# imironhead/ml_super_resolution

Measured on AMD Instinct MI355X. Metric: VDSR-20 training patches/sec (41x41, batch 256 per GPU); fwd HR megapixels/sec alongside, higher is better.
Workload: dtype f32; 1 GPU; BASELINE configs[2]: VDSR 20-layer 3x3x64 residual, RGB, batch 256x41x41 per GPU, fwd+bwd+TF-Adam, random-init weights; global_batch=256, patch=41, parallelism=dp1

## Files before the change

### include/srx.h

```cpp
#ifndef SRX_H_
#define SRX_H_

#include <stddef.h>
#include <stdint.h>

#ifdef __cplusplus
extern "C" {
#endif

typedef void* srx_stream_t;

typedef enum {
    SRX_OK = 0,
    SRX_ERR_BAD_ARG = -1,
    SRX_ERR_UNSUPPORTED = -2,
    SRX_ERR_WORKSPACE = -3,
    SRX_ERR_LAUNCH = -4,
    SRX_ERR_ALIGN = -5
} srx_status;

typedef enum { SRX_PAD_SAME = 0, SRX_PAD_VALID = 1 } srx_pad_mode;

typedef enum {
    SRX_ACT_NONE = 0,
// ... 42 lines not shown
                        const float* x_in, int in_act, float* dx_out, void* ws, size_t ws_bytes,
                        srx_stream_t stream);

int srx_conv2d_bwd_data_acc(const srx_conv_desc* d, const float* dpre, const float* w, const float* dx_acc,
                            float* dx_out, void* ws, size_t ws_bytes, srx_stream_t stream);

int srx_conv2d_bwd_filter(const srx_conv_desc* d, const float* x, const float* dpre, float* dw,
                          float* dbias, const float* w_for_decay, float wd_scale, void* ws,
                          size_t ws_bytes, srx_stream_t stream);

int srx_conv2d_bwd_filter_partials(const srx_conv_desc* d, const float* x, const float* dpre, void* ws,
                                   size_t ws_bytes, int* n_partials, srx_stream_t stream);
int srx_conv2d_bwd_filter_reduce(const srx_conv_desc* d, const void* ws, int n_partials, float* dw,
                                 float* dbias, const float* w_for_decay, float wd_scale,
                                 srx_stream_t stream);

int srx_act_bwd(const float* dy, const float* y, float* dpre, size_t numel, int act,
                srx_stream_t stream);

int srx_depth_to_space(const float* in, float* out, int N, int H, int W, int C, int r,
                       srx_stream_t stream);

int srx_stream_copy(const void* in, void* out, size_t bytes, srx_stream_t stream);

int srx_espcn_forward(const float* x, const float* w1, const float* b1, const float* w2, const float* b2,
                      const float* w3, const float* b3, float* hr, int N, int H, int W, int r,
                      srx_stream_t stream);
int srx_espcn_forward_keep(const float* x, const float* w1, const float* b1, const float* w2, const float* b2,
                           const float* w3, const float* b3, float* t1, float* t2, float* y, int N, int H, int W, int r,
                           srx_stream_t stream);
// ... 139 lines not shown
```

### ml_super_resolution_amd/_lib.py

```python
import ctypes
import os

_HERE = os.path.dirname(os.path.abspath(__file__))
LIB_PATH = os.path.join(_HERE, 'libsrx.so')

SRX_OK = 0
PAD_SAME, PAD_VALID = 0, 1
ACT_NONE, ACT_RELU, ACT_TANH, ACT_LRELU, ACT_SIGMOID = 0, 1, 2, 3, 4
OP_FWD, OP_BWD_DATA, OP_BWD_FILTER = 0, 1, 2
PRECISION_FP32, PRECISION_BF16X3 = 0, 1
PRECISION_BY_NAME = {'highest': PRECISION_FP32, 'high': PRECISION_BF16X3}

ACT_BY_NAME = {None: ACT_NONE, 'none': ACT_NONE, 'relu': ACT_RELU, 'tanh': ACT_TANH,
               'lrelu': ACT_LRELU, 'leaky_relu': ACT_LRELU, 'sigmoid': ACT_SIGMOID}
PAD_BY_NAME = {'same': PAD_SAME, 'valid': PAD_VALID}

EXPORTS = [
    'srx_version', 'srx_last_error', 'srx_set_conv_path', 'srx_set_wgrad_path', 'srx_set_chain', 'srx_conv_chain', 'srx_conv_chain_supported', 'srx_conv2d_precision_supported', 'srx_conv2d_workspace_bytes', 'srx_conv2d_fwd',
    'srx_conv2d_bwd_data', 'srx_conv2d_bwd_filter', 'srx_conv2d_bwd_filter_partials', 'srx_conv2d_bwd_filter_reduce', 'srx_act_bwd', 'srx_depth_to_space',
    'srx_space_to_depth', 'srx_stream_copy', 'srx_mse_fwd_bwd', 'srx_l2_loss', 'srx_reduce_scratch_bytes',
    'srx_adam_tf_step', 'srx_adam_tf_step_dev', 'srx_momentum_clip_step', 'srx_rownorm_loss_fwd_bwd', 'srx_psnr', 'srx_ssim', 'srx_ssim_scratch_bytes', 'srx_saturate_u8', 'srx_affine', 'srx_u8_to_unit_float', 'srx_gaussian_blur', 'srx_resize_bilinear',
    'srx_upsample_nearest', 'srx_upsample_nearest_bwd', 'srx_add_relu_grad',
    'srx_conv2d_bwd_data_acc', 'srx_conv3x3_blocked', 'srx_conv3x3_blocked_bwd_filter_workspace_bytes', 'srx_conv3x3_blocked_bwd_filter',
    'srx_conv3x3_blocked_ex', 'srx_conv3x3_blocked_bwd_filter_ex_workspace_bytes', 'srx_conv3x3_blocked_bwd_filter_ex',
    'srx_espcn_forward', 'srx_espcn_forward_keep', 'srx_debug_poison_lds', 'srx_srcnn_forward', 'srx_maxpool2x2', 'srx_maxpool2x2_bwd', 'srx_maxpool2x2_bwd_masked', 'srx_subsample2', 'srx_subsample2_bwd',
    'srx_channel_blocks_to_nhwc', 'srx_nhwc_to_channel_blocks', 'srx_channel_normalize', 'srx_channel_normalize_bwd',
    'srx_extract_patches16', 'srx_texture_gram', 'srx_texture_gram_bwd', 'srx_pil_resample_ksize', 'srx_pil_resample_coeffs', 'srx_resample_u8', 'srx_u8_to_pm1', 'srx_log_loss', 'srx_vgg_preprocess', 'srx_add_scaled', 'srx_resize_bicubic_tf', 'srx_column_sums', 'srx_gemm_workspace_bytes', 'srx_gemm',
]


class SrxError(RuntimeError):
    pass


# ... 30 lines not shown
    L.srx_last_error.restype = ctypes.c_char_p
    L.srx_set_conv_path.argtypes = [i]
    L.srx_set_wgrad_path.argtypes = [i]
    L.srx_set_chain.argtypes = [i]
    L.srx_conv_chain_supported.argtypes = [dp, i, i]
    L.srx_conv_chain.argtypes = [dp, i, i, i, vp, vp, vp, vp, vp, vp]
    L.srx_conv2d_precision_supported.argtypes = [dp, i]
    L.srx_conv2d_workspace_bytes.argtypes = [dp, i]
    L.srx_conv2d_workspace_bytes.restype = sz
    L.srx_reduce_scratch_bytes.restype = sz
    L.srx_conv2d_fwd.argtypes = [dp, vp, vp, vp, vp, vp, vp, sz, vp]
    L.srx_conv2d_bwd_data.argtypes = [dp, vp, vp, vp, i, vp, vp, sz, vp]
    L.srx_conv2d_bwd_filter.argtypes = [dp, vp, vp, vp, vp, vp, f, vp, sz, vp]
    L.srx_conv2d_bwd_filter_partials.argtypes = [dp, vp, vp, vp, sz, ctypes.POINTER(ctypes.c_int), vp]
    L.srx_conv2d_bwd_filter_reduce.argtypes = [dp, vp, i, vp, vp, vp, f, vp]
    L.srx_act_bwd.argtypes = [vp, vp, vp, sz, i, vp]
    L.srx_depth_to_space.argtypes = [vp, vp, i, i, i, i, i, vp]
    L.srx_space_to_depth.argtypes = [vp, vp, i, i, i, i, i, vp]
    L.srx_stream_copy.argtypes = [vp, vp, sz, vp]
    L.srx_mse_fwd_bwd.argtypes = [vp, vp, sz, f, vp, i, vp, vp, vp]
    L.srx_l2_loss.argtypes = [vp, vp, sz, f, vp, i, vp, vp]
    L.srx_adam_tf_step.argtypes = [vp, vp, vp, vp, sz, f, f, f, f, ctypes.c_int64, f, vp]
    L.srx_adam_tf_step_dev.argtypes = [vp, vp, vp, vp, sz, vp, f, f, f, f, vp]
    L.srx_momentum_clip_step.argtypes = [vp, vp, vp, sz, f, f, f, f, vp]
    L.srx_rownorm_loss_fwd_bwd.argtypes = [vp, vp, sz, sz, vp, vp, vp, vp]
    L.srx_psnr.argtypes = [vp, vp, vp, i, sz, f, vp]
    L.srx_ssim.argtypes = [vp, vp, vp, i, i, i, i, f, vp, vp]
    L.srx_ssim_scratch_bytes.argtypes = [i]
    L.srx_ssim_scratch_bytes.restype = sz
    L.srx_saturate_u8.argtypes = [vp, vp, sz, vp]
# ... 54 lines not shown
```

### ml_super_resolution_amd/csrc/conv_kernels.hip.h

```cpp
#pragma once
#include <hip/hip_runtime.h>
#include <stdint.h>
#include <type_traits>

namespace srx {

typedef float f32x4 __attribute__((ext_vector_type(4)));

enum { ACT_NONE = 0, ACT_RELU = 1, ACT_TANH = 2, ACT_LRELU = 3, ACT_SIGMOID = 4 };

struct ConvArgs {
    const float* x;
    const float* w;
    const float* bias;
    const float* skip;
    const float* mask;
    float* y;
    int N, H, W, OH, OW, Cin, Cout;
    int pad_t, pad_l;
    int TH, TW, NTX, RS;
    int units_total;
    int act, post_relu, mask_act;
    float inv_rs;
    int stagger;
// ... 2441 lines not shown
        }
    }
    bsum += __shfl_xor(bsum, 16);
    bsum += __shfl_xor(bsum, 32);
    if (qpart == 0 && kq == 0 && co_ok) pw[(size_t)TAPS * a.Cin * a.Cout + co] = bsum;
}

template <int IMM>
__device__ __forceinline__ float dpre_fire_imm(__amdgpu_buffer_rsrc_t rsrc, int voff, int soff) {
    float b;
    asm volatile("buffer_load_dword %0, %1, %2, %3 offen offset:%4" : "=&a"(b) : "v"(voff), "s"(rsrc), "s"(soff), "n"(IMM) : "memory");
    return b;
}

template <int KH, int KW, int CINP, int NCH, int OWC>
__global__ __launch_bounds__(256, 1) void wgrad_rows_full_kernel(const WgradArgs a) {
    extern __shared__ __attribute__((aligned(16))) float lds[];
    constexpr int PS = Lds<CINP>::PS;
    constexpr int TAPS = KH * KW;
    constexpr int ROWS = TAPS * CINP;
    constexpr int Q = (ROWS + 63) / 64;
    constexpr int NQP = 4 / NCH;
    constexpr int QW = (Q + NQP - 1) / NQP;
    constexpr int TPP = CINP / 4, PPP = 256 / TPP;
    constexpr int SPR = OWC / 4;
    constexpr int THC = 3;
    constexpr int RSZ = OWC + 1;
    constexpr int COUTC = 64;
    constexpr int U = THC * SPR + 1;
    constexpr int JP = (RSZ + PPP - 1) / PPP;
    constexpr int NPASSES = (THC + KH - 1) * JP;
// ... 44 lines not shown
    SG.m_row = SG.m_last; SG.m_mid = ~0ull;
    const int colb = 16 * COUTC;
    const int lane_b = (kq * COUTC + co_c) * 4;
    const int vb0 = lane_b, vb1 = lane_b + 4 * colb, vb2 = lane_b + 8 * colb;
    const int vX = ((kq * OWC + OWC - 1) * COUTC + co_c) * 4;
    const int rowb = __builtin_amdgcn_readfirstlane(OWC * COUTC * 4);
    const int srow1 = rowb, srow2 = __builtin_amdgcn_readfirstlane(2 * rowb);

    f32x4 acc[QW][4];
#pragma unroll
    for (int k = 0; k < QW; ++k)
#pragma unroll
        for (int g = 0; g < 4; ++g) acc[k][g] = f32x4{0.f, 0.f, 0.f, 0.f};
    float bsum = 0.f;

    const long G_ = gridDim.x;
    const int u0 = (int)(((long)blockIdx.x * a.units_total) / G_);
    const int u1 = (int)(((long)(blockIdx.x + 1) * a.units_total) / G_);

    auto tile_of = [&](int uu_, int& n, int& h, int& th) {
        h = uu_ % a.OH;
        n = uu_ / a.OH;
        th = THC;
        if (a.OH - h < th) th = a.OH - h;
        if (u1 - uu_ < th) th = u1 - uu_;
    };
    auto stage_setup = [&](StageSeq& qi, StageSeq& qc, int h, int th, int buf, bool active) {
        const int left = __builtin_amdgcn_readfirstlane(active ? (th + KH - 1) * JP : 0);
        const int above = (a.pad_t > h) ? (a.pad_t - h) * JP : 0;
        qi.j = 0; qc.j = 0;
        qi.off = __builtin_amdgcn_readfirstlane((h - a.pad_t) * a.W * CINP * 4);
        qc.off = __builtin_amdgcn_readfirstlane(buf * buf_bytes);
        qi.left = left; qc.left = left;
        qi.thr = __builtin_amdgcn_readfirstlane(left - above);
        qc.thr = 0;
    };
    auto x_rsrc = [&](int n) {
        return uniform_rsrc(a.x + ((size_t)n * a.H * a.W - a.pad_l) * CINP, (a.H * a.W + a.pad_l) * CINP * 4);
    };
    auto b_rsrc = [&](int n, int h, int th) {
        return uniform_rsrc(a.dpre + ((size_t)n * a.OH + h) * a.OW * COUTC, th * a.OW * COUTC * 4);
    };

    float bcur[U], bnext[U];
    auto dpre_window_now = [&](__amdgpu_buffer_rsrc_t brs) {
#pragma unroll
        for (int i = 0; i < U; ++i) {
            if (i == U - 1) {
                bnext[i] = __builtin_bit_cast(float, __builtin_amdgcn_raw_buffer_load_b32(brs, vX, 0, 0));
            } else {
                const int r = i / SPR, j = i % SPR;
                const int vb = j < 4 ? vb0 : (j < 8 ? vb1 : vb2);
                bnext[i] = __builtin_bit_cast(float, __builtin_amdgcn_raw_buffer_load_b32(brs, vb + (j % 4) * colb, r * rowb, 0));
            }
        }
    };
// ... 109 lines not shown
        stage_tile_scalar<CINP, 6>(qi, qc, SG, xrs, voff_lane, wl_lane);
        lds_barrier();
        cur_buf ^= 1;
        u = un_;
        t_end += SRX_STAMP() - ts_e;
    }
#undef SRX_TAKE_OVER_B
#ifdef SRX_TRACE
    if (a.trace && lane == 0) {
        unsigned long long* tr = a.trace + ((size_t)blockIdx.x * 4 + wave) * 12;
        tr[0] = t_begin; tr[1] = SRX_STAMP(); tr[2] = t_loop; tr[3] = t_end; tr[4] = 0;
    }
#endif

    asm volatile("s_nop 15\n\ts_nop 7" ::: "memory");
    float* pw = a.part + (size_t)blockIdx.x * a.part_stride;
#pragma unroll
    for (int k = 0; k < QW; ++k) {
        const int q = qpart + k * NQP;
        if (q >= Q) continue;
#pragma unroll
        for (int g = 0; g < 4; ++g) {
#pragma unroll
            for (int r = 0; r < 4; ++r) {
                const int R = 64 * q + 4 * (4 * kq + r) + g;
                const int tap = R / CINP, ci = R % CINP;
                if (R < ROWS && ci < a.Cin && co_ok) pw[((size_t)tap * a.Cin + ci) * a.Cout + co] = acc[k][g][r];
            }
        }
    }
    bsum += __shfl_xor(bsum, 16);
    bsum += __shfl_xor(bsum, 32);
    if (qpart == 0 && kq == 0 && co_ok) pw[(size_t)TAPS * a.Cin * a.Cout + co] = bsum;
}

}
```

### ml_super_resolution_amd/csrc/launchers.h

```cpp
#pragma once
#include "conv_kernels.hip.h"

namespace srx {

struct ConvKey {
    int kh, kw, cinp, nch;
    bool wt;
};

bool launch_conv_k3c64(const ConvKey& k, const ConvArgs& a, int grid, size_t lds, hipStream_t s, hipError_t* err);
bool launch_conv_k3c32(const ConvKey& k, const ConvArgs& a, int grid, size_t lds, hipStream_t s, hipError_t* err);
bool launch_conv_c4(const ConvKey& k, const ConvArgs& a, int grid, size_t lds, hipStream_t s, hipError_t* err);
bool launch_conv_misc(const ConvKey& k, const ConvArgs& a, int grid, size_t lds, hipStream_t s, hipError_t* err);
bool launch_pipe_k3c64(const ConvKey& k, const ConvArgs& a, int grid, size_t lds, hipStream_t s, hipError_t* err);
bool launch_pipe_other(const ConvKey& k, const ConvArgs& a, int grid, size_t lds, hipStream_t s, hipError_t* err);
bool launch_wgrad_narrow(const ConvKey& k, const WgradArgs& a, int grid, hipStream_t s, hipError_t* err);
bool launch_conv_narrow(const ConvKey& k, const ConvArgs& a, hipStream_t s, hipError_t* err);
bool launch_conv_1x1(const ConvKey& k, const ConvArgs& a, long min_pixels, hipStream_t s, hipError_t* err);
bool launch_conv_rows3x3(const ConvKey& k, const ConvArgs& a, long min_pixels, hipStream_t s, hipError_t* err);
bool launch_conv_pack3(const ConvKey& k, const ConvArgs& a, long min_pixels, hipStream_t s, hipError_t* err);
bool launch_conv_kwrows(const ConvKey& k, const ConvArgs& a, long min_pixels, hipStream_t s, hipError_t* err);
bool launch_pipe_strip(const ConvKey& k, const ConvArgs& a, int grid, size_t lds, hipStream_t s, hipError_t* err);
bool launch_conv_generic(const ConvKey& k, const ConvArgs& a, int grid, size_t lds, hipStream_t s, hipError_t* err);
bool launch_wgrad(const ConvKey& k, const WgradArgs& a, int grid, size_t lds, hipStream_t s, hipError_t* err);
bool launch_wgrad_generic(const ConvKey& k, const WgradArgs& a, int grid, size_t lds, hipStream_t s, hipError_t* err);
bool launch_wgrad_lin(const ConvKey& k, const WgradArgs& a, int grid, size_t lds, hipStream_t s, hipError_t* err);
bool launch_wgrad_lin_pack3(const ConvKey& k, const WgradArgs& a, int grid, size_t lds, hipStream_t s, hipError_t* err);
bool launch_wgrad_lin_strip(const ConvKey& k, const WgradArgs& a, int grid, size_t lds, hipStream_t s, hipError_t* err);
bool launch_wgrad_pipe(const ConvKey& k, const WgradArgs& a, int grid, size_t lds, hipStream_t s, hipError_t* err);
bool launch_wgrad_kwcols(const ConvKey& k, const WgradArgs& a, int max_partials, long min_pixels, int* n_partials, hipStream_t s, hipError_t* err);
bool launch_wgrad_1x1(const ConvKey& k, const WgradArgs& a, int max_partials, int* n_partials, hipStream_t s, hipError_t* err);
bool launch_wgrad_rows_full(const ConvKey& k, const WgradArgs& a, int grid, size_t lds, hipStream_t s, hipError_t* err);
bool launch_wgrad_rows_strip(const ConvKey& k, const WgradArgs& a, int grid, size_t lds, hipStream_t s, hipError_t* err);
bool launch_wgrad_lin_pairs(const ConvKey& k, const WgradPairs& q, int grid, int pairs, bool strips, size_t lds, hipStream_t s, hipError_t* err);

__attribute__((weak)) hipError_t launch_conv_chain(bool wt, bool aux, const ConvArgs& a, const ChainPtrs& c, int grid, size_t lds, hipStream_t s);

hipError_t launch_reduce_partials(const float* part, int G, int stride, int wn, int cout, float* dw, float* dbias,
                                  const float* w, float wd, hipStream_t s);
hipError_t launch_reduce_partials_pairs(const float* part, int G, int stride, int wn, int cout, float* dw, float* dbias,
                                        int pairs, int cob, hipStream_t s);

template <typename K, typename A>
inline hipError_t launch_with_lds(K kernel, const A& a, int grid, size_t lds, hipStream_t s, int grid_y = 1) {
    static thread_local const void* configured[64];
    static thread_local int n_configured = 0;
    const void* fn = reinterpret_cast<const void*>(kernel);
    bool known = false;
    for (int i = 0; i < n_configured; ++i) known |= (configured[i] == fn);
    if (!known) {
        hipError_t e = hipFuncSetAttribute(fn, hipFuncAttributeMaxDynamicSharedMemorySize, 160 * 1024);
// ... 98 lines not shown
```

### ml_super_resolution_amd/csrc/srx_api.hip

```cpp
#include <math.h>
#include <stdarg.h>
#include <atomic>
#include <stdio.h>
#include <stdlib.h>
#include <string.h>

#include "../../include/srx.h"
#include "elementwise.h"
#include "launchers.h"
#include "bf16x3.h"

using namespace srx;

namespace {

thread_local char g_err[512] = "";

struct Knobs {
    int pipe_default, narrow, wgrad_lin, wgrad_pipe, wgrad_pipe_strip, wgrad_rows_full, wgrad_1x1, wgrad_pack3, kwrows_min_pixels, big_route_min_pixels, strip_d2s, conv_1x1_min_pixels, pack3_dgrad;
    int chain;
    unsigned long long* trace;
    int dbg;
};
int env_int(const char* name, int dflt) { const char* e = getenv(name); return e ? atoi(e) : dflt; }
Knobs read_knobs() {
    Knobs k;
    k.pipe_default = env_int("SRX_PIPE", 1);
    k.narrow = env_int("SRX_NARROW", 1);
    k.wgrad_lin = env_int("SRX_WGRAD_LIN", 1);
    k.wgrad_pipe = env_int("SRX_WGRAD_PIPE", 1);
    k.wgrad_pipe_strip = env_int("SRX_WGRAD_PIPE_STRIP", 1);
    k.kwrows_min_pixels = env_int("SRX_KWROWS_MIN_PIXELS", 4096);
    k.big_route_min_pixels = env_int("SRX_BIG_ROUTE_MIN_PIXELS", 60000);
    k.conv_1x1_min_pixels = env_int("SRX_CONV_1X1_MIN_PIXELS", 100000);
    k.pack3_dgrad = env_int("SRX_PACK3_DGRAD", 1);
    k.strip_d2s = env_int("SRX_STRIP_D2S", 1);
    k.wgrad_rows_full = env_int("SRX_WGRAD_ROWS_FULL", 1);
    k.wgrad_1x1 = env_int("SRX_WGRAD_1X1", 1);
    k.wgrad_pack3 = env_int("SRX_WGRAD_PACK3", 1);
    k.chain = env_int("SRX_CHAIN", 1);
    k.trace = nullptr;
    k.dbg = 0;
#ifdef SRX_TRACE
    { const char* tp = getenv("SRX_TRACE_PTR"); k.trace = tp ? (unsigned long long*)strtoull(tp, nullptr, 0) : nullptr; }
    k.dbg = env_int("SRX_DBG", 0);
#endif
    return k;
}
const Knobs& knobs() { static const Knobs k = read_knobs(); return k; }

std::atomic<int> g_use_pipe{-1};
std::atomic<int> g_chain{-1};
int use_chain() { const int v = g_chain.load(std::memory_order_relaxed); return v < 0 ? (knobs().chain ? 1 : 0) : v; }
int use_pipe() { const int v = g_use_pipe.load(std::memory_order_relaxed); return v < 0 ? knobs().pipe_default : v; }
std::atomic<int> g_wgrad_path{-1};
int wgrad_path_default() { return !knobs().wgrad_lin ? 0 : ((knobs().wgrad_pipe || knobs().wgrad_pipe_strip) ? 2 : 1); }
int wgrad_path() { const int v = g_wgrad_path.load(std::memory_order_relaxed); return v < 0 ? wgrad_path_default() : v; }

int cu_count() {
    static std::atomic<int> cached[64];
    int dev = 0;
    if (hipGetDevice(&dev) != hipSuccess || dev < 0 || dev >= 64) { (void)hipGetLastError(); return 256; }
    int n = cached[dev].load(std::memory_order_relaxed);
    if (n > 0) return n;
    if (hipDeviceGetAttribute(&n, hipDeviceAttributeMultiprocessorCount, dev) != hipSuccess || n <= 0) {
        (void)hipGetLastError();
        n = 256;
    }
// ... 661 lines not shown
                                            w_for_decay, wd_scale, (hipStream_t)stream);
    if (err != hipSuccess) return fail(SRX_ERR_LAUNCH, "reduce launch failed: %s", hipGetErrorString(err));
    return SRX_OK;
}

int srx_conv2d_bwd_filter(const srx_conv_desc* d, const float* x, const float* dpre, float* dw, float* dbias,
                          const float* w_for_decay, float wd_scale, void* ws, size_t ws_bytes, srx_stream_t stream) {
    if (!dw) return fail(SRX_ERR_BAD_ARG, "null tensor pointer");
    int n = 0;
    const int rc = srx_conv2d_bwd_filter_partials(d, x, dpre, ws, ws_bytes, &n, stream);
    if (rc) return rc;
    return srx_conv2d_bwd_filter_reduce(d, ws, n, dw, dbias, w_for_decay, wd_scale, stream);
}

namespace {
void blocked_desc(srx_conv_desc* d, int N, int H, int W) {
    memset(d, 0, sizeof(*d));
    d->N = N; d->H = H; d->W = W; d->Cin = 64; d->Cout = 64; d->KH = 3; d->KW = 3; d->stride = 1; d->pad_mode = SRX_PAD_SAME;
}
int pairs_route(const srx_conv_desc* d, const Plan& p, int pairs, int* G, size_t* lin_lds) {
    *lin_lds = p.lds_bytes + 4 * (size_t)(p.cinp + 4) * 4;
    const bool common = wgrad_path() >= 1 && p.cinp == 64 && p.nch == 4 && d->W >= 4 && p.RS >= 8 && *lin_lds <= 80 * 1024 &&
                        (long)d->H * d->W * 64 * 4 < (1L << 31) - 4096;
    const bool lin_ok = common && p.NTX == 1 && p.RS == d->W + p.pad_l && (long)p.TH * d->W * 64 * 4 < (1L << 30);
    const int wppp = 256 / (64 / 4);
    const bool strip_ok = common && p.NTX > 1 && p.RS >= wppp && p.TW >= 4 && (d->W % p.TW == 0 || d->W % p.TW >= 4) &&
                          p.RS <= 3 * wppp && (long)d->H * d->W * 64 * 4 < (1L << 30);
    int g = max_grid() / pairs;
    if (g < 1) g = 1;
    if (g > p.grid) g = p.grid;
// ... 313 lines not shown
```

### ml_super_resolution_amd/engine.py

```python
import math
import os

import torch

from . import ops


class LayerSpec(object):

    def __init__(self, ksize, cin, cout, padding='same', act=None, scope=None):
        self.kh, self.kw = (ksize, ksize) if isinstance(ksize, int) else ksize
        self.cin, self.cout = cin, cout
        self.padding = padding.lower()
        self.act = act
        self.scope = scope

    @property
    def kernel_shape(self):
        return (self.kh, self.kw, self.cin, self.cout)

    def out_hw(self, h, w):
        if self.padding == 'same':
            return h, w
        return h - self.kh + 1, w - self.kw + 1
# ... 163 lines not shown
            j += 1
        return j

    def _dgrad_chain(self, acts):
        last = len(self.specs) - 1
        for hi in range(last - 1, 0, -1):
            s = self.specs[hi]
            lo = hi
            while (lo >= 1 and hi - lo < 32 and self.specs[lo].padding == s.padding and self.specs[lo - 1].act == self.specs[hi - 1].act and
                   tuple(acts[lo].shape) == tuple(acts[hi].shape) and self._chain_ok(lo, acts[lo].shape, ops._lib.OP_BWD_DATA)):
                lo -= 1
            if hi - lo >= 2:
                return lo + 1, hi
        return None

    def loss_and_backward(self, target, numel_global=None):
        if self._acts is None:
            raise RuntimeError('forward(keep=True) must run before loss_and_backward')
        acts = self._acts
        y = acts[-1]
        last = len(self.specs) - 1
        inv = 1.0 / (y.numel() if numel_global is None else numel_global)
        if self.loss_kind == 'rownorm':
            row_len = y.shape[1] * y.shape[2]
            dy = ops.rownorm_loss_fwd_bwd(y, target, row_len, self.loss, dpred=self._buf(('dy', 0), y.shape),
                                          norms=self._buf(('rownorms',), (y.numel() // row_len,)))
        else:
            dy = self._buf(('dy', 0), y.shape)
            ops.mse_fwd_bwd(y, target, self.loss, inv_numel=inv, accumulate=False, dpred=dy)
        if self.weight_decay:
            self.add_regulariser_loss()
        if self.specs[last].act is not None:
            dpre = ops.act_bwd(dy, y, self.specs[last].act, out=self._buf(('dpre_last',), y.shape))
        else:
            dpre = dy
        prec = self.layer_precision
        need = max(ops.bwd_filter_workspace_bytes(acts[i].shape, s.kernel_shape, s.padding, precision=prec[i])
                   for i, s in enumerate(self.specs))
        if self._ws is None or self._ws.numel() * 4 < need:
            self._step_graphs.clear()
            self._ws = torch.empty((need + 3) // 4, dtype=torch.float32, device=self.device)
        chain = self._dgrad_chain(acts)
        for i in range(last, -1, -1):
            s = self.specs[i]
            if chain is not None and chain[0] <= i <= chain[1]:
                lo, hi = chain
                if i == hi:
                    outs = [self._buf(('dpre_chain', k - 1), acts[k].shape) for k in range(hi, lo - 1, -1)]
                    ops.conv2d_bwd_data_chain([dpre] + outs[:-1], [self.kernel(k) for k in range(hi, lo - 1, -1)],
                                              [acts[k] for k in range(hi, lo - 1, -1)], outs, acts[hi].shape, s.padding,
                                              in_act=self.specs[hi - 1].act)
                    dpres = {hi: dpre}
                    for k in range(hi, lo - 1, -1):
                        dpres[k - 1] = outs[hi - k]
                ops.conv2d_bwd_filter(acts[i], dpres[i], s.kernel_shape, s.padding,
                                      w_for_decay=self.kernel(i) if self.weight_decay else None,
                                      wd_scale=self.weight_decay, dw=self.kernel(i, self.grads),
                                      dbias=self.bias(i, self.grads), workspace=self._ws, precision=prec[i])
                if i == lo:
                    dpre = dpres[lo - 1]
                continue
            ops.conv2d_bwd_filter(acts[i], dpre, s.kernel_shape, s.padding,
                                  w_for_decay=self.kernel(i) if self.weight_decay else None,
                                  wd_scale=self.weight_decay, dw=self.kernel(i, self.grads),
                                  dbias=self.bias(i, self.grads), workspace=self._ws, precision=prec[i])
            if i > 0:
                prev_act = self.specs[i - 1].act
                out = self._buf(('dx', i % 3, acts[i].shape[3]), acts[i].shape)
                dpre = ops.conv2d_bwd_data(dpre, self.kernel(i), acts[i].shape, s.padding,
                                           x_in=acts[i] if prev_act is not None else None, in_act=prev_act, out=out,
                                           precision=prec[i])
        if self.grad_hook is not None:
            self.grad_hook(self.grads)
        return self.loss

    def add_regulariser_loss(self):
        if self._decay_mask is None:
            self._decay_mask = torch.zeros_like(self.params)
            for k_off, kn, _, _ in self.slices:
                self._decay_mask[k_off:k_off + kn] = 1.0
        ops.l2_loss(self.params, self.weight_decay, self.loss, accumulate=True, mask=self._decay_mask)

    def adam_step(self, lr, beta1=0.9, beta2=0.999, eps=1e-8):
# ... 53 lines not shown
            if ent['warm'] < 2:
                ent['warm'] += 1
                loss = eager(x, target)
                if key not in self._step_graphs:
                    self._step_graphs[key] = ent
                return loss
            if self.opt_m is None:
                self.opt_m = torch.zeros_like(self.params)
                if momentum is None:
                    self.opt_v = torch.zeros_like(self.params)
            if momentum is None:
                self._sync_adam_state(lr)
            sx, st = x.clone(), target.clone()
            torch.cuda.synchronize(self.device)
            g = torch.cuda.CUDAGraph()
            with torch.cuda.graph(g):
                self.forward(sx, keep=True)
                self.loss_and_backward(st)
                optimizer_launch()
            ent.update(graph=g, x=sx, t=st)
        if momentum is None:
            self._sync_adam_state(lr)
        if x.data_ptr() != ent['x'].data_ptr():
            ent['x'].copy_(x)
        if target.data_ptr() != ent['t'].data_ptr():
            ent['t'].copy_(target)
        ent['graph'].replay()
        self.global_step += 1
        if momentum is None:
            self._state_t += 1
        return self.loss
# ... 122 lines not shown
```

### ml_super_resolution_amd/espcn/model_espcn.py

```python
import os

import numpy as np
import torch

from .. import graph, ops
from ..engine import ConvStack, LayerSpec, truncated_normal_


def layer_specs(scaling_factor=3):
    r2 = scaling_factor * scaling_factor
    return [LayerSpec(5, 3, 64, 'same', 'tanh', 'f1'),
            LayerSpec(3, 64, 32, 'same', 'tanh', 'f2'),
            LayerSpec(3, 32, 3 * r2, 'same', None, 'f3')]


class EspcnModel(object):
    def __init__(self, scaling_factor=3, device='cuda', seed=None):
        self.scaling_factor = scaling_factor
        self.stack = ConvStack(layer_specs(scaling_factor), device=device, residual=False, weight_decay=0.0)
        gen = torch.Generator().manual_seed(seed) if seed is not None else None
        for i in range(3):
            truncated_normal_(self.stack.kernel(i), 0.02, gen)
        self.placeholders = {}
        self.use_graph = os.environ.get('SRX_ESPCN_GRAPH', '1') != '0'
# ... 58 lines not shown
        if len(self._graphs) >= 8:
            self._graphs.pop(next(iter(self._graphs)))
        static_in = lr_source.clone()
        n, h, w, _ = lr_source.shape
        r = self.scaling_factor
        out = torch.empty((n, h * r, w * r, 3), dtype=torch.float32, device=lr_source.device)
        mids = (torch.empty((n, h, w, 64), dtype=torch.float32, device=lr_source.device),
                torch.empty((n, h, w, 32), dtype=torch.float32, device=lr_source.device))
        side = torch.cuda.Stream(device=lr_source.device)
        side.wait_stream(torch.cuda.current_stream(lr_source.device))
        with torch.cuda.stream(side):
            for _ in range(2):
                self._super_resolve_launches(static_in, out=out, mids=mids)
        torch.cuda.current_stream(lr_source.device).wait_stream(side)
        graph_obj = torch.cuda.CUDAGraph()
        with torch.cuda.graph(graph_obj):
            self._super_resolve_launches(static_in, out=out, mids=mids)
        return static_in, graph_obj, out, mids

    def train_step(self, lr_source, hr_target, learning_rate):
        return self.stack.train_step_replay(lr_source, hr_target, learning_rate)

    def save(self, path):
        arrays = {k + ':0': v.detach().cpu().numpy() for k, v in self.stack.variables().items()}
        arrays['global_step'] = np.int64(self.stack.global_step)
        np.savez(path, **arrays)

    def run(self, keys, feed_dict):
        dev = self.stack.device
        feeds = {name: feed_dict[ph] for name, ph in self.placeholders.items() if ph in feed_dict}
        needs_forward = [k for k in keys if k != 'step']
# ... 77 lines not shown
```

### ml_super_resolution_amd/ops.py

```python
import ctypes
import os

import torch

from . import _lib
from ._lib import ACT_BY_NAME, PAD_BY_NAME, ConvDesc, check
from ._lib import lib as _load_lib

_POISON_LDS = os.environ.get('SRX_POISON_LDS', '0') == '1'


def lib():
    L = _load_lib()
    if _POISON_LDS and torch.cuda.is_available():
        L.srx_debug_poison_lds(_stream())
    return L



def _stream():
    return ctypes.c_void_p(torch.cuda.current_stream().cuda_stream)


def _ptr(t):
# ... 151 lines not shown
    _chk(x, 'x'); _chk(dpre, 'dpre'); _chk(workspace, 'workspace')
    d = conv_desc(x.shape, w_shape, padding, precision=precision)
    n = ctypes.c_int(0)
    check(lib().srx_conv2d_bwd_filter_partials(ctypes.byref(d), _ptr(x), _ptr(dpre), _ptr(workspace), workspace.numel() * 4,
                                               ctypes.byref(n), _stream()), 'srx_conv2d_bwd_filter_partials')
    return n.value


def conv2d_bwd_filter_reduce(x_shape, w_shape, padding, workspace, n_partials, dw, dbias=None, w_for_decay=None, wd_scale=0.0,
                             precision='highest'):
    _chk(workspace, 'workspace'); _chk(dw, 'dw')
    d = conv_desc(x_shape, w_shape, padding, precision=precision)
    check(lib().srx_conv2d_bwd_filter_reduce(ctypes.byref(d), _ptr(workspace), int(n_partials), _ptr(dw), _ptr(dbias),
                                             _ptr(w_for_decay), float(wd_scale), _stream()), 'srx_conv2d_bwd_filter_reduce')
    return dw, dbias


def act_bwd(dy, y, act, out=None):
    _chk(dy, 'dy'); _chk(y, 'y')
    out = out if out is not None else torch.empty_like(dy)
    check(lib().srx_act_bwd(_ptr(dy), _ptr(y), _ptr(out), dy.numel(), ACT_BY_NAME[act], _stream()), 'srx_act_bwd')
    return out


def depth_to_space(x, r, out=None):
    _chk(x, 'x')
    N, H, W, D = x.shape
    if D % (r * r):
        raise ValueError('depth %d not divisible by r*r=%d' % (D, r * r))
    C = D // (r * r)
# ... 509 lines not shown
```

Baseline: 18920 patches/s.

## Batch filter-gradient kernels of multiple 3x3 64->64 layers into one launch

Adds a batched weight-gradient path that computes the filter gradients of several consecutive identical 3x3 64->64 layers in one kernel launch. The grid is split across layers, and a single reduce kernel sums the per-workgroup partials and applies weight decay for every layer. The backward loop keeps each layer's dpre in a dedicated buffer until the lowest layer in the batch is reached, then launches once. This is meant to cut per-layer launch and tail underutilisation for the 41-wide rows kernel, at the cost of keeping more dpre buffers alive and fewer workgroups per layer.

```diff
diff --git a/include/srx.h b/include/srx.h
--- a/include/srx.h
+++ b/include/srx.h
@@ -80,6 +80,13 @@
 int srx_conv2d_bwd_filter_reduce(const srx_conv_desc* d, const void* ws, int n_partials, float* dw,
                                  float* dbias, const float* w_for_decay, float wd_scale,
                                  srx_stream_t stream);
+
+int srx_conv2d_bwd_filter_batch(const srx_conv_desc* d, int n_layers, const float* const* x, const float* const* dpre,
+                                float* const* dw, float* const* dbias, const float* const* w_for_decay, float wd_scale,
+                                void* ws, size_t ws_bytes, srx_stream_t stream);
+size_t srx_conv2d_bwd_filter_batch_workspace_bytes(const srx_conv_desc* d, int n_layers);
+int srx_conv2d_bwd_filter_batch_plan(const srx_conv_desc* d, int n_layers, int* wgs_per_layer, int* grid);
+int srx_set_wgrad_batch(int on);
 
 int srx_act_bwd(const float* dy, const float* y, float* dpre, size_t numel, int act,
                 srx_stream_t stream);
diff --git a/ml_super_resolution_amd/_lib.py b/ml_super_resolution_amd/_lib.py
--- a/ml_super_resolution_amd/_lib.py
+++ b/ml_super_resolution_amd/_lib.py
@@ -17,7 +17,8 @@
 
 EXPORTS = [
     'srx_version', 'srx_last_error', 'srx_set_conv_path', 'srx_set_wgrad_path', 'srx_set_chain', 'srx_conv_chain', 'srx_conv_chain_supported', 'srx_conv2d_precision_supported', 'srx_conv2d_workspace_bytes', 'srx_conv2d_fwd',
-    'srx_conv2d_bwd_data', 'srx_conv2d_bwd_filter', 'srx_conv2d_bwd_filter_partials', 'srx_conv2d_bwd_filter_reduce', 'srx_act_bwd', 'srx_depth_to_space',
+    'srx_conv2d_bwd_data', 'srx_conv2d_bwd_filter', 'srx_conv2d_bwd_filter_partials', 'srx_conv2d_bwd_filter_reduce',
+    'srx_conv2d_bwd_filter_batch', 'srx_conv2d_bwd_filter_batch_workspace_bytes', 'srx_conv2d_bwd_filter_batch_plan', 'srx_set_wgrad_batch', 'srx_act_bwd', 'srx_depth_to_space',
     'srx_space_to_depth', 'srx_stream_copy', 'srx_mse_fwd_bwd', 'srx_l2_loss', 'srx_reduce_scratch_bytes',
     'srx_adam_tf_step', 'srx_adam_tf_step_dev', 'srx_momentum_clip_step', 'srx_rownorm_loss_fwd_bwd', 'srx_psnr', 'srx_ssim', 'srx_ssim_scratch_bytes', 'srx_saturate_u8', 'srx_affine', 'srx_u8_to_unit_float', 'srx_gaussian_blur', 'srx_resize_bilinear',
     'srx_upsample_nearest', 'srx_upsample_nearest_bwd', 'srx_add_relu_grad',
@@ -78,6 +79,11 @@
     L.srx_conv2d_bwd_filter.argtypes = [dp, vp, vp, vp, vp, vp, f, vp, sz, vp]
     L.srx_conv2d_bwd_filter_partials.argtypes = [dp, vp, vp, vp, sz, ctypes.POINTER(ctypes.c_int), vp]
     L.srx_conv2d_bwd_filter_reduce.argtypes = [dp, vp, i, vp, vp, vp, f, vp]
+    L.srx_conv2d_bwd_filter_batch.argtypes = [dp, i, vp, vp, vp, vp, vp, f, vp, sz, vp]
+    L.srx_conv2d_bwd_filter_batch_workspace_bytes.argtypes = [dp, i]
+    L.srx_conv2d_bwd_filter_batch_workspace_bytes.restype = sz
+    L.srx_conv2d_bwd_filter_batch_plan.argtypes = [dp, i, ctypes.POINTER(ctypes.c_int), ctypes.POINTER(ctypes.c_int)]
+    L.srx_set_wgrad_batch.argtypes = [i]
     L.srx_act_bwd.argtypes = [vp, vp, vp, sz, i, vp]
     L.srx_depth_to_space.argtypes = [vp, vp, i, i, i, i, i, vp]
     L.srx_space_to_depth.argtypes = [vp, vp, i, i, i, i, i, vp]
diff --git a/ml_super_resolution_amd/csrc/conv_kernels.hip.h b/ml_super_resolution_amd/csrc/conv_kernels.hip.h
--- a/ml_super_resolution_amd/csrc/conv_kernels.hip.h
+++ b/ml_super_resolution_amd/csrc/conv_kernels.hip.h
@@ -2479,7 +2479,8 @@
 }
 
 template <int KH, int KW, int CINP, int NCH, int OWC>
-__global__ __launch_bounds__(256, 1) void wgrad_rows_full_kernel(const WgradArgs a) {
+__device__ __forceinline__ void wgrad_rows_full_body(const WgradArgs& a, const float* __restrict__ x, const float* __restrict__ dpre,
+                                                     float* __restrict__ pw, const int u0, const int u1) {
     extern __shared__ __attribute__((aligned(16))) float lds[];
     constexpr int PS = Lds<CINP>::PS;
     constexpr int TAPS = KH * KW;
@@ -2554,10 +2555,6 @@
         for (int g = 0; g < 4; ++g) acc[k][g] = f32x4{0.f, 0.f, 0.f, 0.f};
     float bsum = 0.f;
 
-    const long G_ = gridDim.x;
-    const int u0 = (int)(((long)blockIdx.x * a.units_total) / G_);
-    const int u1 = (int)(((long)(blockIdx.x + 1) * a.units_total) / G_);
-
     auto tile_of = [&](int uu_, int& n, int& h, int& th) {
         h = uu_ % a.OH;
         n = uu_ / a.OH;
@@ -2576,10 +2573,10 @@
         qc.thr = 0;
     };
     auto x_rsrc = [&](int n) {
-        return uniform_rsrc(a.x + ((size_t)n * a.H * a.W - a.pad_l) * CINP, (a.H * a.W + a.pad_l) * CINP * 4);
+        return uniform_rsrc(x + ((size_t)n * a.H * a.W - a.pad_l) * CINP, (a.H * a.W + a.pad_l) * CINP * 4);
     };
     auto b_rsrc = [&](int n, int h, int th) {
-        return uniform_rsrc(a.dpre + ((size_t)n * a.OH + h) * a.OW * COUTC, th * a.OW * COUTC * 4);
+        return uniform_rsrc(dpre + ((size_t)n * a.OH + h) * a.OW * COUTC, th * a.OW * COUTC * 4);
     };
 
     float bcur[U], bnext[U];
@@ -2719,7 +2716,6 @@
 #endif
 
     asm volatile("s_nop 15\n\ts_nop 7" ::: "memory");
-    float* pw = a.part + (size_t)blockIdx.x * a.part_stride;
 #pragma unroll
     for (int k = 0; k < QW; ++k) {
         const int q = qpart + k * NQP;
@@ -2739,4 +2735,31 @@
     if (qpart == 0 && kq == 0 && co_ok) pw[(size_t)TAPS * a.Cin * a.Cout + co] = bsum;
 }
 
-}
+template <int KH, int KW, int CINP, int NCH, int OWC>
+__global__ __launch_bounds__(256, 1) void wgrad_rows_full_kernel(const WgradArgs a) {
+    const long G_ = gridDim.x;
+    const int u0 = (int)(((long)blockIdx.x * a.units_total) / G_);
+    const int u1 = (int)(((long)(blockIdx.x + 1) * a.units_total) / G_);
+    wgrad_rows_full_body<KH, KW, CINP, NCH, OWC>(a, a.x, a.dpre, a.part + (size_t)blockIdx.x * a.part_stride, u0, u1);
+}
+
+struct WgradBatchPtrs {
+    const float* x[kChainMax];
+    const float* dpre[kChainMax];
+};
+struct WgradBatchOut {
+    float* dw[kChainMax];
+    float* dbias[kChainMax];
+    const float* w[kChainMax];
+};
+
+template <int KH, int KW, int CINP, int NCH, int OWC>
+__global__ __launch_bounds__(256, 1) void wgrad_rows_batch_kernel(const WgradArgs a, const WgradBatchPtrs c, const int wpl) {
+    const int layer = __builtin_amdgcn_readfirstlane((int)blockIdx.x / wpl);
+    const int sub = (int)blockIdx.x - layer * wpl;
+    const int u0 = (int)(((long)sub * a.units_total) / wpl);
+    const int u1 = (int)(((long)(sub + 1) * a.units_total) / wpl);
+    wgrad_rows_full_body<KH, KW, CINP, NCH, OWC>(a, c.x[layer], c.dpre[layer], a.part + (size_t)blockIdx.x * a.part_stride, u0, u1);
+}
+
+}
diff --git a/ml_super_resolution_amd/csrc/launchers.h b/ml_super_resolution_amd/csrc/launchers.h
--- a/ml_super_resolution_amd/csrc/launchers.h
+++ b/ml_super_resolution_amd/csrc/launchers.h
@@ -35,6 +35,10 @@
 bool launch_wgrad_lin_pairs(const ConvKey& k, const WgradPairs& q, int grid, int pairs, bool strips, size_t lds, hipStream_t s, hipError_t* err);
 
 __attribute__((weak)) hipError_t launch_conv_chain(bool wt, bool aux, const ConvArgs& a, const ChainPtrs& c, int grid, size_t lds, hipStream_t s);
+
+__attribute__((weak)) hipError_t launch_wgrad_rows_batch(const WgradArgs& a, const WgradBatchPtrs& c, int wpl, int layers, size_t lds, hipStream_t s);
+__attribute__((weak)) hipError_t launch_wgrad_batch_reduce(const float* part, int wpl, int layers, int stride, int wn, int cout,
+                                                           const WgradBatchOut& o, float wd, hipStream_t s);
 
 hipError_t launch_reduce_partials(const float* part, int G, int stride, int wn, int cout, float* dw, float* dbias,
                                   const float* w, float wd, hipStream_t s);
diff --git a/ml_super_resolution_amd/csrc/srx_api.hip b/ml_super_resolution_amd/csrc/srx_api.hip
--- a/ml_super_resolution_amd/csrc/srx_api.hip
+++ b/ml_super_resolution_amd/csrc/srx_api.hip
@@ -18,7 +18,7 @@
 
 struct Knobs {
     int pipe_default, narrow, wgrad_lin, wgrad_pipe, wgrad_pipe_strip, wgrad_rows_full, wgrad_1x1, wgrad_pack3, kwrows_min_pixels, big_route_min_pixels, strip_d2s, conv_1x1_min_pixels, pack3_dgrad;
-    int chain;
+    int chain, wgrad_batch;
     unsigned long long* trace;
     int dbg;
 };
@@ -39,6 +39,7 @@
     k.wgrad_1x1 = env_int("SRX_WGRAD_1X1", 1);
     k.wgrad_pack3 = env_int("SRX_WGRAD_PACK3", 1);
     k.chain = env_int("SRX_CHAIN", 1);
+    k.wgrad_batch = env_int("SRX_WGRAD_BATCH", 1);
     k.trace = nullptr;
     k.dbg = 0;
 #ifdef SRX_TRACE
@@ -52,6 +53,8 @@
 std::atomic<int> g_use_pipe{-1};
 std::atomic<int> g_chain{-1};
 int use_chain() { const int v = g_chain.load(std::memory_order_relaxed); return v < 0 ? (knobs().chain ? 1 : 0) : v; }
+std::atomic<int> g_wgrad_batch{-1};
+int use_wgrad_batch() { const int v = g_wgrad_batch.load(std::memory_order_relaxed); return v < 0 ? (knobs().wgrad_batch ? 1 : 0) : v; }
 int use_pipe() { const int v = g_use_pipe.load(std::memory_order_relaxed); return v < 0 ? knobs().pipe_default : v; }
 std::atomic<int> g_wgrad_path{-1};
 int wgrad_path_default() { return !knobs().wgrad_lin ? 0 : ((knobs().wgrad_pipe || knobs().wgrad_pipe_strip) ? 2 : 1); }
@@ -743,6 +746,99 @@
 }
 
 namespace {
+int wgrad_batch_plan(const srx_conv_desc* d, int layers, WgradArgs* a, int* wpl, int* grid) {
+    int rc = check_desc(d);
+    if (rc) return rc;
+    if (!use_wgrad_batch()) return fail(SRX_ERR_UNSUPPORTED, "bwd_filter_batch: switched off (srx_set_wgrad_batch / SRX_WGRAD_BATCH)");
+    if (!launch_wgrad_rows_batch || !launch_wgrad_batch_reduce) return fail(SRX_ERR_UNSUPPORTED, "bwd_filter_batch: this build has no batch kernels");
+    if (layers < 2 || layers > kChainMax) return fail(SRX_ERR_UNSUPPORTED, "bwd_filter_batch: %d layers (2..%d)", layers, kChainMax);
+    if (d->precision != SRX_PRECISION_FP32) return fail(SRX_ERR_UNSUPPORTED, "bwd_filter_batch: precision %d (exact fp32 only)", d->precision);
+    if (d->KH != 3 || d->KW != 3 || d->Cin != 64 || d->Cout != 64 || d->stride != 1 || d->pad_mode != SRX_PAD_SAME)
+        return fail(SRX_ERR_UNSUPPORTED, "bwd_filter_batch: only 3x3 64->64 stride-1 SAME layers");
+    if (d->W != 41) return fail(SRX_ERR_UNSUPPORTED, "bwd_filter_batch: W %d (only 41-pixel rows: wgrad_rows_full_kernel's shape)", d->W);
+    if (wgrad_path() < 2 || !knobs().wgrad_pipe || !knobs().wgrad_rows_full)
+        return fail(SRX_ERR_UNSUPPORTED, "bwd_filter_batch: the filter-gradient path is not wgrad_rows_full_kernel's (srx_set_wgrad_path)");
+    int pt, pl, OH, OW;
+    geometry(d, &pt, &pl, &OH, &OW);
+    Plan p;
+    rc = make_plan(d->N, d->H, d->W, OH, OW, d->Cin, d->Cout, d->KH, d->KW, pt, pl, &p);
+    if (rc) return rc;
+    wgrad_tile_for_linear_walk(d, &p);
+    const bool ok = p.NTX == 1 && p.RS == 42 && pl == 1 && pt == 1 && OW == 41 && (long)d->H * d->W * d->Cin * 4 < (1L << 31) - 4096;
+    if (!ok) return fail(SRX_ERR_UNSUPPORTED, "bwd_filter_batch: the shape is not on wgrad_rows_full_kernel's route");
+    const long rows = (long)d->N * OH;
+    long w = pipe_grid() / layers;
+    if (w > rows) w = rows;
+    if (w < 1) return fail(SRX_ERR_UNSUPPORTED, "bwd_filter_batch: %d layers on a grid of %d", layers, pipe_grid());
+    *wpl = (int)w;
+    *grid = pipe_grid();
+    memset(a, 0, sizeof(*a));
+    a->part_stride = (int)part_stride(d);
+    a->N = d->N; a->H = d->H; a->W = d->W; a->OH = OH; a->OW = OW; a->Cin = d->Cin; a->Cout = d->Cout;
+    a->pad_t = pt; a->pad_l = pl; a->TH = 3; a->TW = p.TW; a->NTX = p.NTX; a->RS = p.RS;
+    a->units_total = p.units_total; a->inv_rs = 1.0f / (float)p.RS;
+    a->stride = 1;
+    a->zero_slot = (3 + 3) * 42 + 2;
+    return SRX_OK;
+}
+}
+
+int srx_set_wgrad_batch(int on) {
+    const int old = g_wgrad_batch.exchange(on < 0 ? -1 : (on ? 1 : 0), std::memory_order_relaxed);
+    return old < 0 ? (knobs().wgrad_batch ? 1 : 0) : old;
+}
+
+int srx_conv2d_bwd_filter_batch_plan(const srx_conv_desc* d, int n_layers, int* wgs_per_layer, int* grid) {
+    WgradArgs a;
+    int wpl = 0, g = 0;
+    const int rc = wgrad_batch_plan(d, n_layers, &a, &wpl, &g);
+    if (rc) { wpl = 0; g = 0; }
+    if (wgs_per_layer) *wgs_per_layer = wpl;
+    if (grid) *grid = g;
+    return rc;
+}
+
+size_t srx_conv2d_bwd_filter_batch_workspace_bytes(const srx_conv_desc* d, int n_layers) {
+    WgradArgs a;
+    int wpl = 0, g = 0;
+    if (wgrad_batch_plan(d, n_layers, &a, &wpl, &g) != SRX_OK) return 0;
+    return (size_t)n_layers * wpl * part_stride(d) * sizeof(float);
+}
+
+int srx_conv2d_bwd_filter_batch(const srx_conv_desc* d, int n_layers, const float* const* x, const float* const* dpre, float* const* dw,
+                                float* const* dbias, const float* const* w_for_decay, float wd_scale, void* ws, size_t ws_bytes,
+                                srx_stream_t stream) {
+    WgradArgs a;
+    int wpl = 0, g = 0;
+    int rc = wgrad_batch_plan(d, n_layers, &a, &wpl, &g);
+    if (rc) return rc;
+    if (!x || !dpre || !dw) return fail(SRX_ERR_BAD_ARG, "null pointer array");
+    WgradBatchPtrs c;
+    WgradBatchOut o;
+    memset(&c, 0, sizeof(c));
+    memset(&o, 0, sizeof(o));
+    for (int l = 0; l < n_layers; ++l) {
+        if (!x[l] || !dpre[l] || !dw[l]) return fail(SRX_ERR_BAD_ARG, "bwd_filter_batch: null tensor pointer in layer %d", l);
+        float* const db = dbias ? dbias[l] : nullptr;
+        const float* const wl = w_for_decay ? w_for_decay[l] : nullptr;
+        if (!aligned16(x[l]) || !aligned16(dpre[l]) || !aligned16(dw[l]) || (db && !aligned16(db)) || (wl && !aligned16(wl)))
+            return fail(SRX_ERR_UNSUPPORTED, "bwd_filter_batch: layer %d: every pointer must be 16-byte aligned", l);
+        c.x[l] = x[l]; c.dpre[l] = dpre[l];
+        o.dw[l] = dw[l]; o.dbias[l] = db; o.w[l] = wl;
+    }
+    const size_t need = (size_t)n_layers * wpl * part_stride(d) * sizeof(float);
+    if (!ws || ws_bytes < need) return fail(SRX_ERR_WORKSPACE, "bwd_filter_batch needs %zu workspace bytes, got %zu", need, ws_bytes);
+    if (!aligned16(ws)) return fail(SRX_ERR_UNSUPPORTED, "bwd_filter_batch: the workspace must be 16-byte aligned");
+    a.part = (float*)ws;
+    hipError_t err = launch_wgrad_rows_batch(a, c, wpl, n_layers, 2 * (size_t)(a.zero_slot + 4) * (64 + 4) * 4, (hipStream_t)stream);
+    if (err != hipSuccess) return fail(SRX_ERR_LAUNCH, "wgrad batch launch failed: %s", hipGetErrorString(err));
+    err = launch_wgrad_batch_reduce((const float*)ws, wpl, n_layers, a.part_stride, d->KH * d->KW * d->Cin * d->Cout, d->Cout, o, wd_scale,
+                                    (hipStream_t)stream);
+    if (err != hipSuccess) return fail(SRX_ERR_LAUNCH, "reduce launch failed: %s", hipGetErrorString(err));
+    return SRX_OK;
+}
+
+namespace {
 void blocked_desc(srx_conv_desc* d, int N, int H, int W) {
     memset(d, 0, sizeof(*d));
     d->N = N; d->H = H; d->W = W; d->Cin = 64; d->Cout = 64; d->KH = 3; d->KW = 3; d->stride = 1; d->pad_mode = SRX_PAD_SAME;
diff --git a/ml_super_resolution_amd/csrc/wgrad_batch.hip b/ml_super_resolution_amd/csrc/wgrad_batch.hip
--- /dev/null
+++ b/ml_super_resolution_amd/csrc/wgrad_batch.hip
@@ -0,0 +1,52 @@
+#include "launchers.h"
+namespace srx {
+
+__global__ __launch_bounds__(256) void wgrad_batch_reduce_kernel(const float* __restrict__ part, const int wpl, const int stride,
+                                                                 const int wn, const int n, const WgradBatchOut o, const float wd) {
+    const int layer = blockIdx.y;
+    const int j = (blockIdx.x * 256 + threadIdx.x) * 4;
+    if (j >= n) return;
+    const float* p = part + (size_t)layer * wpl * stride + j;
+    f32x4 s = {0.f, 0.f, 0.f, 0.f};
+    int g = 0;
+    for (; g + 8 <= wpl; g += 8) {
+        f32x4 v[8];
+#pragma unroll
+        for (int i = 0; i < 8; ++i) v[i] = *reinterpret_cast<const f32x4*>(p + (size_t)(g + i) * stride);
+#pragma unroll
+        for (int i = 0; i < 8; ++i) s += v[i];
+    }
+    for (; g < wpl; ++g) s += *reinterpret_cast<const f32x4*>(p + (size_t)g * stride);
+    float* __restrict__ dw = o.dw[layer];
+    float* __restrict__ dbias = o.dbias[layer];
+    const float* __restrict__ w = o.w[layer];
+#pragma unroll
+    for (int e = 0; e < 4; ++e) {
+        const int jj = j + e;
+        if (jj < wn)
+            dw[jj] = s[e] + (w ? wd * w[jj] : 0.f);
+        else if (jj < n && dbias)
+            dbias[jj - wn] = s[e];
+    }
+}
+
+hipError_t launch_wgrad_rows_batch(const WgradArgs& a, const WgradBatchPtrs& c, int wpl, int layers, size_t lds, hipStream_t s) {
+    static thread_local bool configured = false;
+    const void* fn = reinterpret_cast<const void*>(wgrad_rows_batch_kernel<3, 3, 64, 4, 41>);
+    if (!configured) {
+        hipError_t e = hipFuncSetAttribute(fn, hipFuncAttributeMaxDynamicSharedMemorySize, 160 * 1024);
+        if (e != hipSuccess) return e;
+        configured = true;
+    }
+    hipLaunchKernelGGL((wgrad_rows_batch_kernel<3, 3, 64, 4, 41>), dim3((unsigned)(wpl * layers)), dim3(256), lds, s, a, c, wpl);
+    return hipGetLastError();
+}
+
+hipError_t launch_wgrad_batch_reduce(const float* part, int wpl, int layers, int stride, int wn, int cout, const WgradBatchOut& o,
+                                     float wd, hipStream_t s) {
+    const int n = wn + cout;
+    hipLaunchKernelGGL(wgrad_batch_reduce_kernel, dim3((unsigned)((n + 1023) / 1024), (unsigned)layers), dim3(256), 0, s, part, wpl,
+                       stride, wn, n, o, wd);
+    return hipGetLastError();
+}
+}
diff --git a/ml_super_resolution_amd/engine.py b/ml_super_resolution_amd/engine.py
--- a/ml_super_resolution_amd/engine.py
+++ b/ml_super_resolution_amd/engine.py
@@ -1,9 +1,24 @@
+import contextlib
+import gc
 import math
 import os
 
 import torch
 
 from . import ops
+
+
+@contextlib.contextmanager
+def capture_graph(g):
+    gc.collect()
+    was_enabled = gc.isenabled()
+    gc.disable()
+    try:
+        with torch.cuda.graph(g):
+            yield
+    finally:
+        if was_enabled:
+            gc.enable()
 
 
 class LayerSpec(object):
@@ -201,6 +216,22 @@
                 return lo + 1, hi
         return None
 
+    def _wgrad_batch(self, acts):
+        best = None
+        i, n = 0, len(self.specs)
+        while i < n:
+            s = self.specs[i]
+            j = i
+            while (j < n and j - i < 32 and self.layer_precision[j] == 'highest' and self.specs[j].kernel_shape == s.kernel_shape and
+                   self.specs[j].padding == s.padding and tuple(acts[j].shape) == tuple(acts[i].shape) and
+                   tuple(acts[j + 1].shape) == tuple(acts[i + 1].shape)):
+                j += 1
+            if j - i >= 2 and (best is None or j - i > best[1] - best[0] + 1):
+                if ops.bwd_filter_batch_plan(acts[i].shape, s.kernel_shape, j - i, s.padding)[0] > 0:
+                    best = (i, j - 1)
+            i = max(j, i + 1)
+        return best
+
     def loss_and_backward(self, target, numel_global=None):
         if self._acts is None:
             raise RuntimeError('forward(keep=True) must run before loss_and_backward')
@@ -224,10 +255,34 @@
         prec = self.layer_precision
         need = max(ops.bwd_filter_workspace_bytes(acts[i].shape, s.kernel_shape, s.padding, precision=prec[i])
                    for i, s in enumerate(self.specs))
+        batch = self._wgrad_batch(acts)
+        if batch is not None:
+            b_lo, b_hi = batch
+            need = max(need, ops.bwd_filter_batch_workspace_bytes(acts[b_lo].shape, self.specs[b_lo].kernel_shape, b_hi - b_lo + 1,
+                                                                  self.specs[b_lo].padding))
         if self._ws is None or self._ws.numel() * 4 < need:
             self._step_graphs.clear()
             self._ws = torch.empty((need + 3) // 4, dtype=torch.float32, device=self.device)
         chain = self._dgrad_chain(acts)
+        in_batch = lambda k: batch is not None and batch[0] <= k <= batch[1]
+        dpres = {}
+
+        def wgrad(i, dpre_i):
+            s = self.specs[i]
+            if not in_batch(i):
+                ops.conv2d_bwd_filter(acts[i], dpre_i, s.kernel_shape, s.padding,
+                                      w_for_decay=self.kernel(i) if self.weight_decay else None,
+                                      wd_scale=self.weight_decay, dw=self.kernel(i, self.grads),
+                                      dbias=self.bias(i, self.grads), workspace=self._ws, precision=prec[i])
+                return
+            dpres[i] = dpre_i
+            if i == batch[0]:
+                ks = list(range(batch[0], batch[1] + 1))
+                ops.conv2d_bwd_filter_batch([acts[k] for k in ks], [dpres[k] for k in ks], [self.kernel(k, self.grads) for k in ks],
+                                            [self.bias(k, self.grads) for k in ks],
+                                            [self.kernel(k) for k in ks] if self.weight_decay else None, self.weight_decay,
+                                            s.padding, workspace=self._ws)
+
         for i in range(last, -1, -1):
             s = self.specs[i]
             if chain is not None and chain[0] <= i <= chain[1]:
@@ -237,23 +292,18 @@
                     ops.conv2d_bwd_data_chain([dpre] + outs[:-1], [self.kernel(k) for k in range(hi, lo - 1, -1)],
                                               [acts[k] for k in range(hi, lo - 1, -1)], outs, acts[hi].shape, s.padding,
                                               in_act=self.specs[hi - 1].act)
-                    dpres = {hi: dpre}
+                    cdpres = {hi: dpre}
                     for k in range(hi, lo - 1, -1):
-                        dpres[k - 1] = outs[hi - k]
-                ops.conv2d_bwd_filter(acts[i], dpres[i], s.kernel_shape, s.padding,
-                                      w_for_decay=self.kernel(i) if self.weight_decay else None,
-                                      wd_scale=self.weight_decay, dw=self.kernel(i, self.grads),
-                                      dbias=self.bias(i, self.grads), workspace=self._ws, precision=prec[i])
+                        cdpres[k - 1] = outs[hi - k]
+                wgrad(i, cdpres[i])
                 if i == lo:
-                    dpre = dpres[lo - 1]
+                    dpre = cdpres[lo - 1]
                 continue
-            ops.conv2d_bwd_filter(acts[i], dpre, s.kernel_shape, s.padding,
-                                  w_for_decay=self.kernel(i) if self.weight_decay else None,
-                                  wd_scale=self.weight_decay, dw=self.kernel(i, self.grads),
-                                  dbias=self.bias(i, self.grads), workspace=self._ws, precision=prec[i])
+            wgrad(i, dpre)
             if i > 0:
                 prev_act = self.specs[i - 1].act
-                out = self._buf(('dx', i % 3, acts[i].shape[3]), acts[i].shape)
+                out = (self._buf(('dpre_chain', i - 1), acts[i].shape) if in_batch(i - 1)
+                       else self._buf(('dx', i % 3, acts[i].shape[3]), acts[i].shape))
                 dpre = ops.conv2d_bwd_data(dpre, self.kernel(i), acts[i].shape, s.padding,
                                            x_in=acts[i] if prev_act is not None else None, in_act=prev_act, out=out,
                                            precision=prec[i])
@@ -337,7 +387,7 @@
             sx, st = x.clone(), target.clone()
             torch.cuda.synchronize(self.device)
             g = torch.cuda.CUDAGraph()
-            with torch.cuda.graph(g):
+            with capture_graph(g):
                 self.forward(sx, keep=True)
                 self.loss_and_backward(st)
                 optimizer_launch()
diff --git a/ml_super_resolution_amd/espcn/model_espcn.py b/ml_super_resolution_amd/espcn/model_espcn.py
--- a/ml_super_resolution_amd/espcn/model_espcn.py
+++ b/ml_super_resolution_amd/espcn/model_espcn.py
@@ -4,7 +4,7 @@
 import torch
 
 from .. import graph, ops
-from ..engine import ConvStack, LayerSpec, truncated_normal_
+from ..engine import ConvStack, LayerSpec, capture_graph, truncated_normal_
 
 
 def layer_specs(scaling_factor=3):
@@ -96,7 +96,7 @@
                 self._super_resolve_launches(static_in, out=out, mids=mids)
         torch.cuda.current_stream(lr_source.device).wait_stream(side)
         graph_obj = torch.cuda.CUDAGraph()
-        with torch.cuda.graph(graph_obj):
+        with capture_graph(graph_obj):
             self._super_resolve_launches(static_in, out=out, mids=mids)
         return static_in, graph_obj, out, mids
 
diff --git a/ml_super_resolution_amd/ops.py b/ml_super_resolution_amd/ops.py
--- a/ml_super_resolution_amd/ops.py
+++ b/ml_super_resolution_amd/ops.py
@@ -189,6 +189,45 @@
     check(lib().srx_conv2d_bwd_filter_reduce(ctypes.byref(d), _ptr(workspace), int(n_partials), _ptr(dw), _ptr(dbias),
                                              _ptr(w_for_decay), float(wd_scale), _stream()), 'srx_conv2d_bwd_filter_reduce')
     return dw, dbias
+
+
+def bwd_filter_batch_plan(x_shape, w_shape, n_layers, padding='same', stride=1, precision='highest'):
+    d = conv_desc(x_shape, w_shape, padding, stride=stride, precision=precision)
+    wpl, grid = ctypes.c_int(0), ctypes.c_int(0)
+    _load_lib().srx_conv2d_bwd_filter_batch_plan(ctypes.byref(d), int(n_layers), ctypes.byref(wpl), ctypes.byref(grid))
+    return wpl.value, grid.value
+
+
+def bwd_filter_batch_workspace_bytes(x_shape, w_shape, n_layers, padding='same', stride=1, precision='highest'):
+    d = conv_desc(x_shape, w_shape, padding, stride=stride, precision=precision)
+    return _load_lib().srx_conv2d_bwd_filter_batch_workspace_bytes(ctypes.byref(d), int(n_layers))
+
+
+def conv2d_bwd_filter_batch(xs, dpres, dws, dbiases=None, w_for_decay=None, wd_scale=0.0, padding='same', workspace=None,
+                            stride=1, precision='highest'):
+    L = len(xs)
+    if not (len(dpres) == len(dws) == L) or (dbiases is not None and len(dbiases) != L) or (w_for_decay is not None and len(w_for_decay) != L):
+        raise ValueError('conv2d_bwd_filter_batch: the per-layer lists differ in length')
+    for l in range(L):
+        _chk(xs[l], 'x'); _chk(dpres[l], 'dpre'); _chk(dws[l], 'dw')
+        _chk(None if dbiases is None else dbiases[l], 'dbias'); _chk(None if w_for_decay is None else w_for_decay[l], 'w_for_decay')
+    d = conv_desc(xs[0].shape, dws[0].shape, padding, stride=stride, precision=precision)
+    for l in range(L):
+        if tuple(xs[l].shape) != tuple(xs[0].shape) or tuple(dpres[l].shape) != tuple(out_shape(d)) or tuple(dws[l].shape) != tuple(dws[0].shape):
+            raise ValueError('conv2d_bwd_filter_batch: layer %d does not have the shape of layer 0' % l)
+    if workspace is None:
+        need = _load_lib().srx_conv2d_bwd_filter_batch_workspace_bytes(ctypes.byref(d), L)
+        workspace = torch.empty((max(need, 16) + 3) // 4, dtype=torch.float32, device=xs[0].device)
+    _chk(workspace, 'workspace')
+    check(lib().srx_conv2d_bwd_filter_batch(ctypes.byref(d), L, _ptr_array(xs), _ptr_array(dpres), _ptr_array(dws),
+                                            None if dbiases is None else _ptr_array(dbiases),
+                                            None if w_for_decay is None else _ptr_array(w_for_decay), float(wd_scale),
+                                            _ptr(workspace), workspace.numel() * 4, _stream()), 'srx_conv2d_bwd_filter_batch')
+    return dws, dbiases
+
+
+def set_wgrad_batch(on):
+    return lib().srx_set_wgrad_batch(int(on))
 
 
 def act_bwd(dy, y, act, out=None):
```

New measurement: 19420 patches/s (median of 6 runs). +2.6%, better.
